# haoxiangsnr/Wave-U-Net-for-Speech-Enhancement

Measured on AMD Instinct MI355X. Metric: 16384-sample frames/sec fwd+bwd, 12-level Wave-U-Net, higher is better.
Workload: dtype f32 (levels >= 16 samples: 3 x f16 MFMA on hi/lo fp16 halves, fp32 accumulate; the rest f32 MFMA); 1 GPU; unet_basic 12-level, 16384-sample frames, batch=64 per GPU, fp32, training-mode forward + smooth_l1 + backward + fused HIP Adam step (BASELINE.json configs[2]; configs[3] when n_gpus>1); global_batch=64, frame=16384, parallelism=dp1

## Files before the change

### wave-u-net-for-speech-enhancement_amd/csrc/wunet_elementwise.h

```cpp
#pragma once
#include "wunet_dev.h"

struct PackDesc {
    const float* w;
    float* dst;
    int Cout, Cin, taps;
    int M;
    int CP;
    int mtiles;
    int transposed;
};

#define WUNET_MAX_CONV_LAYERS 34
struct PackTable { PackDesc d[WUNET_MAX_CONV_LAYERS]; };

static __global__ __launch_bounds__(WUNET_THREADS) void pack_weights_kernel(PackTable tab)
{
    const PackDesc& d = tab.d[blockIdx.y];
    const int total = d.mtiles * d.CP * d.taps * 16;
    const int kc = d.transposed ? d.Cout : d.Cin;
    for (int idx = blockIdx.x * WUNET_THREADS + threadIdx.x; idx < total; idx += gridDim.x * WUNET_THREADS) {
        const int i = idx & 15;
        int r = idx >> 4;
        const int t = r % d.taps; r /= d.taps;
        const int c = r % d.CP;
        const int mt = r / d.CP;
        const int m = mt * 16 + i;
        float v = 0.0f;
        if (m < d.M && c < kc) {
            v = d.transposed ? d.w[((size_t)c * d.Cin + m) * d.taps + (d.taps - 1 - t)]
                             : d.w[((size_t)m * d.Cin + c) * d.taps + t];
        }
        d.dst[idx] = v;
    }
}

template <int N>
__device__ __forceinline__ void block_sum(double (&a)[N], double* red)
{
    const int tid = threadIdx.x;
#pragma unroll
    for (int m = 32; m > 0; m >>= 1) {
#pragma unroll
        for (int k = 0; k < N; ++k) a[k] += wunet_shfl_xor_d(a[k], m);
    }
    __syncthreads();
    if ((tid & 63) == 0) {
#pragma unroll
        for (int k = 0; k < N; ++k) red[k * WUNET_WAVES + (tid >> 6)] = a[k];
    }
    __syncthreads();
#pragma unroll
    for (int k = 0; k < N; ++k)
        a[k] = (red[k * WUNET_WAVES] + red[k * WUNET_WAVES + 1]) + (red[k * WUNET_WAVES + 2] + red[k * WUNET_WAVES + 3]);
}

__device__ __forceinline__ void block_sum2(double& a, double& b, double* red)
{
    double v[2] = {a, b};
    block_sum<2>(v, red);
    a = v[0]; b = v[1];
}

struct RowPiece { size_t row, piece, beg, end; };
__device__ __forceinline__ RowPiece row_piece(size_t row, size_t piece, size_t plen, size_t len)
{
    const size_t beg = piece * plen;
    return RowPiece{row, piece, beg, beg + plen < len ? beg + plen : len};
}

__device__ __forceinline__ void block_max2(float& a, float& b, double* red)
{
    float* fr = reinterpret_cast<float*>(red);
    const int tid = threadIdx.x;
#pragma unroll
    for (int m = 32; m > 0; m >>= 1) {
        a = fmaxf(a, wunet_shfl_xor(a, m));
        b = fmaxf(b, wunet_shfl_xor(b, m));
    }
    __syncthreads();
    if ((tid & 63) == 0) {
        fr[tid >> 6] = a;
        fr[WUNET_WAVES + (tid >> 6)] = b;
    }
    __syncthreads();
    a = fmaxf(fmaxf(fr[0], fr[1]), fmaxf(fr[2], fr[3]));
    b = fmaxf(fmaxf(fr[WUNET_WAVES], fr[WUNET_WAVES + 1]), fmaxf(fr[WUNET_WAVES + 2], fr[WUNET_WAVES + 3]));
}

struct BnFwdArgs {
    const float* stats;
    int rows;
    const float* bias;
    const float* gamma;
    const float* beta;
    float* running_mean;
    float* running_var;
    long long* nbt;
    float* a;
    float* s;
    float* mean;
    float* rstd;
    int C;
    double count;
    int training;
};

struct BnFwdPre { float bias, gamma, beta, rmean, rvar; long long nbt; };
__device__ __forceinline__ BnFwdPre bn_finalize_preload(const BnFwdArgs& A, int c)
{
    BnFwdPre P;
    P.bias = A.bias[c]; P.gamma = A.gamma[c]; P.beta = A.beta[c]; P.rmean = A.running_mean[c]; P.rvar = A.running_var[c];
    P.nbt = c == 0 ? *A.nbt : 0;
    return P;
}
__device__ __forceinline__ void bn_finalize_core(const BnFwdArgs& A, int c, double s1, double s2, const BnFwdPre& P)
{
    const double m0 = s1 / A.count;
    double var = s2 / A.count - m0 * m0;
    var = var < 0.0 ? 0.0 : var;
    const double mean = m0 + (double)P.bias;
    const float rstd = (float)(1.0 / sqrt(var + 1e-5));
    const float a = P.gamma * rstd;
    const float sh = P.beta - (float)mean * a;
    A.a[c] = a;
    A.s[c] = sh;
    A.mean[c] = (float)mean;
    A.rstd[c] = rstd;
    const double unbiased = A.count > 1.0 ? var * A.count / (A.count - 1.0) : var;
    A.running_mean[c] = (float)(0.9 * (double)P.rmean + 0.1 * mean);
    A.running_var[c] = (float)(0.9 * (double)P.rvar + 0.1 * unbiased);
    if (c == 0) *A.nbt = P.nbt + 1;
}

__device__ __forceinline__ void bn_eval_core(const BnFwdArgs& A, int c)
{
    const float rstd = (float)(1.0 / sqrt((double)A.running_var[c] + 1e-5));
    const float a = A.gamma[c] * rstd;
    A.a[c] = a;
    A.s[c] = A.beta[c] - A.running_mean[c] * a;
}

struct BnEvalDesc { const float* gamma; const float* beta; const float* running_mean; const float* running_var; float* a; float* s; int C;
                    float* mean; float* rstd; };
struct BnEvalTable { BnEvalDesc d[WUNET_MAX_CONV_LAYERS]; };
static __global__ __launch_bounds__(WUNET_THREADS) void bn_eval_all_kernel(BnEvalTable T)
{
    const BnEvalDesc& d = T.d[blockIdx.y];
    const int c = blockIdx.x * WUNET_THREADS + threadIdx.x;
    if (c >= d.C) return;
    BnFwdArgs A{};
    A.gamma = d.gamma; A.beta = d.beta; A.running_mean = const_cast<float*>(d.running_mean); A.running_var = const_cast<float*>(d.running_var);
    A.a = d.a; A.s = d.s;
    bn_eval_core(A, c);
    if (d.mean) {
        const float rstd = (float)(1.0 / sqrt((double)d.running_var[c] + 1e-5)), a = d.gamma[c] * rstd;
        const float mu = d.running_mean[c], sh = d.beta[c] - mu * a;
        d.mean[c] = mu;
        d.rstd[c] = rstd;
    }
}

static __global__ __launch_bounds__(WUNET_THREADS) void bn_finalize_fwd_kernel(BnFwdArgs A)
{
    __shared__ double red[2 * WUNET_THREADS];
    const int c = blockIdx.x, tid = threadIdx.x;
    if (!A.training) {
        if (tid == 0) bn_eval_core(A, c);
        return;
    }
    const BnFwdPre P = bn_finalize_preload(A, c);
    double s1 = 0.0, s2 = 0.0;
    const float2* st = reinterpret_cast<const float2*>(A.stats) + (size_t)c * A.rows;
    int r = tid;
    for (; r + 3 * WUNET_THREADS < A.rows; r += 4 * WUNET_THREADS) {
        const float2 v0 = st[r], v1 = st[r + WUNET_THREADS], v2 = st[r + 2 * WUNET_THREADS], v3 = st[r + 3 * WUNET_THREADS];
        s1 += (double)v0.x; s2 += (double)v0.y;
        s1 += (double)v1.x; s2 += (double)v1.y;
        s1 += (double)v2.x; s2 += (double)v2.y;
        s1 += (double)v3.x; s2 += (double)v3.y;
    }
    for (; r < A.rows; r += WUNET_THREADS) {
        const float2 v = st[r];
        s1 += (double)v.x;
        s2 += (double)v.y;
    }
    block_sum2(s1, s2, red);
    if (tid == 0) bn_finalize_core(A, c, s1, s2, P);
}

__device__ __forceinline__ wunet_f4 wunet_sum_splits4(const float* p, int ksplit, size_t stride)
{
    wunet_f4 v = wunet_f4{0.f, 0.f, 0.f, 0.f};
    int k = 0;
    for (; k + 4 <= ksplit; k += 4) {
        const wunet_f4 t0 = wunet_ld4(p + (size_t)k * stride), t1 = wunet_ld4(p + (size_t)(k + 1) * stride);
        const wunet_f4 t2 = wunet_ld4(p + (size_t)(k + 2) * stride), t3 = wunet_ld4(p + (size_t)(k + 3) * stride);
#pragma unroll
        for (int j = 0; j < 4; ++j) { v[j] += t0[j]; v[j] += t1[j]; v[j] += t2[j]; v[j] += t3[j]; }
    }
    for (; k < ksplit; ++k) {
        const wunet_f4 t = wunet_ld4(p + (size_t)k * stride);
#pragma unroll
        for (int j = 0; j < 4; ++j) v[j] += t[j];
    }
    return v;
}

static __global__ __launch_bounds__(WUNET_THREADS) void conv_reduce_bn_kernel(BnFwdArgs A, const float* part, int ksplit,
                                                                        size_t split_stride, float* z, int B, int L, int logL,
                                                                        float* stats_rows, int Lt, float* xb)
{
    __shared__ double red[2 * WUNET_THREADS];
    const int c = blockIdx.x, tid = threadIdx.x;
    const float bias = A.bias[c];
    double s1 = 0.0, s2 = 0.0;
    const int total = B * L;
    if (!A.training) {
        const float ea = xb ? A.a[c] : 0.0f, es = xb ? A.s[c] : 0.0f;
        float m = 0.0f, m2 = 0.0f;
        if ((L & 3) == 0) {
            const int total4 = total >> 2;
            const int per = (total4 + gridDim.y - 1) / gridDim.y;
            const int beg = blockIdx.y * per, end = beg + per < total4 ? beg + per : total4;
            for (int p4 = beg + tid; p4 < end; p4 += WUNET_THREADS) {
                const int p = p4 << 2;
                const int b = p >> logL, l = p & (L - 1);
                const size_t off = ((size_t)b * A.C + c) * L + l;
                const wunet_f4 v = wunet_sum_splits4(part + off, ksplit, split_stride);
                wunet_f4 o;
#pragma unroll
                for (int j = 0; j < 4; ++j) {
                    o[j] = v[j] + bias;
                    m = fmaxf(m, fabsf(ea * o[j] + es));
                }
                wunet_st4(z + off, o);
            }
        } else {
            const int per = (total + gridDim.y - 1) / gridDim.y;
            const int beg = blockIdx.y * per, end = beg + per < total ? beg + per : total;
            for (int p = beg + tid; p < end; p += WUNET_THREADS) {
                const int b = p >> logL, l = p & (L - 1);
                const size_t off = ((size_t)b * A.C + c) * L + l;
                float v = 0.0f;
                for (int k = 0; k < ksplit; ++k) v += part[(size_t)k * split_stride + off];
                z[off] = v + bias;
                m = fmaxf(m, fabsf(ea * (v + bias) + es));
            }
        }
        if (xb) {
            block_max2(m, m2, red);
            if (tid == 0) wunet_atomic_absmax(xb, m);
        }
        return;
    }
    BnFwdPre P{};
    if (gridDim.y == 1) P = bn_finalize_preload(A, c);
    if ((L & 3) == 0) {
        const int total4 = total >> 2;
        const int per = (total4 + gridDim.y - 1) / gridDim.y;
        const int beg = blockIdx.y * per, end = beg + per < total4 ? beg + per : total4;
        for (int p4 = beg + tid; p4 < end; p4 += WUNET_THREADS) {
            const int p = p4 << 2;
            const int b = p >> logL, l = p & (L - 1);
            const size_t off = ((size_t)b * A.C + c) * L + l;
            const wunet_f4 v = wunet_sum_splits4(part + off, ksplit, split_stride);
            wunet_f4 o;
#pragma unroll
            for (int j = 0; j < 4; ++j) {
                o[j] = v[j] + bias;
                if (l + j < Lt) {
                    s1 += (double)v[j];
                    s2 += (double)v[j] * (double)v[j];
                }
            }
            wunet_st4(z + off, o);
        }
    } else {
        const int per = (total + gridDim.y - 1) / gridDim.y;
        const int beg = blockIdx.y * per, end = beg + per < total ? beg + per : total;
        for (int p = beg + tid; p < end; p += WUNET_THREADS) {
            const int b = p >> logL, l = p & (L - 1);
            const size_t off = ((size_t)b * A.C + c) * L + l;
            float v = 0.0f;
            for (int k = 0; k < ksplit; ++k) v += part[(size_t)k * split_stride + off];
            z[off] = v + bias;
            if (l < Lt) {
                s1 += (double)v;
                s2 += (double)v * (double)v;
            }
        }
    }
    block_sum2(s1, s2, red);
    if (tid == 0) {
        if (gridDim.y > 1) {
            float* st = stats_rows + ((size_t)c * gridDim.y + blockIdx.y) * 2;
            st[0] = (float)s1;
            st[1] = (float)s2;
        } else bn_finalize_core(A, c, s1, s2, P);
    }
}

static __global__ __launch_bounds__(WUNET_THREADS) void split_sum_kernel(const float* part, int ksplit, size_t n, float* out,
                                                                   const float* bias, int C, int logL)
{
    if ((n & 3) == 0 && (bias == nullptr || logL >= 2)) {
        const size_t n4 = n >> 2;
        for (size_t i4 = (size_t)blockIdx.x * WUNET_THREADS + threadIdx.x; i4 < n4; i4 += (size_t)gridDim.x * WUNET_THREADS) {
            const size_t i = i4 << 2;
            wunet_f4 v = wunet_sum_splits4(part + i, ksplit, n);
            const float bv = bias ? bias[(i >> logL) % (size_t)C] : 0.0f;
#pragma unroll
            for (int j = 0; j < 4; ++j) v[j] += bv;
            wunet_st4(out + i, v);
        }
        return;
    }
    for (size_t i = (size_t)blockIdx.x * WUNET_THREADS + threadIdx.x; i < n; i += (size_t)gridDim.x * WUNET_THREADS) {
        float v = 0.0f;
        for (int k = 0; k < ksplit; ++k) v += part[(size_t)k * n + i];
        out[i] = v + (bias ? bias[(i >> logL) % (size_t)C] : 0.0f);
    }
}

struct HeadFwdArgs {
    const float* z;
    const float* a;
    const float* s;
    const float* in;
    const float* wh;
    const float* bh;
    float* out;
    int B, C, T, logT;
};

static __global__ __launch_bounds__(WUNET_THREADS) void head_fwd_kernel(HeadFwdArgs A)
{
    const size_t total4 = ((size_t)A.B * A.T) >> 2;
    const float bh = A.bh[0], win = A.wh[A.C];
    for (size_t q4 = (size_t)blockIdx.x * WUNET_THREADS + threadIdx.x; q4 < total4; q4 += (size_t)gridDim.x * WUNET_THREADS) {
        const size_t p = q4 << 2;
        const size_t b = p >> A.logT, t = p & (size_t)(A.T - 1);
        const float* zr = A.z + b * A.C * A.T + t;
        const wunet_f4 xin = wunet_ld4(A.in + p);
        wunet_f4 acc = wunet_f4{bh, bh, bh, bh};
        int c = 0;
        for (; c + 24 <= A.C; c += 24) {
            wunet_f4 v[24];
#pragma unroll
            for (int e = 0; e < 24; ++e) v[e] = wunet_ld4(zr + (size_t)(c + e) * A.T);
#pragma unroll
            for (int e = 0; e < 24; ++e) {
                const float av = A.a[c + e], sv = A.s[c + e], wv = A.wh[c + e];
#pragma unroll
                for (int j = 0; j < 4; ++j) acc[j] += wv * wunet_lrelu(av * v[e][j] + sv);
            }
        }
        for (; c + 8 <= A.C; c += 8) {
            wunet_f4 v[8];
#pragma unroll
            for (int e = 0; e < 8; ++e) v[e] = wunet_ld4(zr + (size_t)(c + e) * A.T);
#pragma unroll
            for (int e = 0; e < 8; ++e) {
                const float av = A.a[c + e], sv = A.s[c + e], wv = A.wh[c + e];
#pragma unroll
                for (int j = 0; j < 4; ++j) acc[j] += wv * wunet_lrelu(av * v[e][j] + sv);
            }
        }
        for (; c < A.C; ++c) {
            const wunet_f4 v = wunet_ld4(zr + (size_t)c * A.T);
            const float av = A.a[c], sv = A.s[c], wv = A.wh[c];
#pragma unroll
            for (int j = 0; j < 4; ++j) acc[j] += wv * wunet_lrelu(av * v[j] + sv);
        }
        wunet_f4 o;
#pragma unroll
        for (int j = 0; j < 4; ++j) o[j] = tanhf(acc[j] + win * xin[j]);
        wunet_st4(A.out + p, o);
    }
}

struct HeadBwdArgs {
    const float* z; const float* a; const float* s; const float* in;
    const float* out; const float* gout;
    float* gh;
    float* part;
    int B, C, T, logT;
};

static __global__ __launch_bounds__(WUNET_THREADS) void head_bwd_kernel(HeadBwdArgs A)
{
    __shared__ double red[2 * WUNET_THREADS];
    const size_t total = (size_t)A.B * A.T;
    const size_t per = (total + gridDim.x - 1) / gridDim.x;
    const size_t beg = (size_t)blockIdx.x * per, end = beg + per < total ? beg + per : total;
    double sb = 0.0, sin_ = 0.0;
    size_t p = beg + threadIdx.x;
    for (; p + 3 * WUNET_THREADS < end; p += 4 * WUNET_THREADS) {
        float o[4], go[4], xi[4];
#pragma unroll
        for (int u = 0; u < 4; ++u) { o[u] = A.out[p + u * WUNET_THREADS]; go[u] = A.gout[p + u * WUNET_THREADS]; xi[u] = A.in[p + u * WUNET_THREADS]; }
#pragma unroll
        for (int u = 0; u < 4; ++u) {
            const float g = go[u] * (1.0f - o[u] * o[u]);
            A.gh[p + u * WUNET_THREADS] = g;
            sb += (double)g;
            sin_ += (double)g * (double)xi[u];
        }
    }
    for (; p < end; p += WUNET_THREADS) {
        const float o = A.out[p];
        const float g = A.gout[p] * (1.0f - o * o);
        A.gh[p] = g;
        sb += (double)g;
        sin_ += (double)g * (double)A.in[p];
    }
    block_sum2(sb, sin_, red);
    if (threadIdx.x == 0) {
        A.part[(size_t)blockIdx.x * 2] = (float)sin_;
        A.part[(size_t)blockIdx.x * 2 + 1] = (float)sb;
    }
}

static __global__ __launch_bounds__(WUNET_THREADS) void rows_sum_kernel(const float* part, int rows, int n, float* out0, int n0, float* out1)
{
    __shared__ double red[2 * WUNET_THREADS];
    const int j = blockIdx.x;
    double s = 0.0, dummy = 0.0;
    for (int r = threadIdx.x; r < rows; r += WUNET_THREADS) s += (double)part[(size_t)r * n + j];
    block_sum2(s, dummy, red);
    if (threadIdx.x == 0) {
        if (j < n0) out0[j] = (float)s; else out1[j - n0] = (float)s;
    }
}

struct BnBwdArgs {
    const float* part; int rows;
    const float* gamma; const float* mean; const float* rstd;
    float* dgamma; float* dbeta;
    float* dbias;
    float* k1; float* k2; float* k3;
    int C; double count;
    const float* pmax;
    float* bound;
    const float* e0rows;
    float* dw0;
    int frozen;
};

struct BnBwdFold { float k1, k2, k3, dgamma, dbeta, dbias, bound; };
__device__ __forceinline__ BnBwdFold bn_bwd_fold(float gamma, float rstd, float mean, double s1, double s2, double count, int frozen, float mg, float mz)
{
    const double m1 = frozen ? 0.0 : s1 / count, m2 = frozen ? 0.0 : s2 / count;
    const double a = (double)gamma * (double)rstd;
    BnBwdFold f;
    f.k1 = (float)a;
    f.k2 = (float)(-a * m2 * (double)rstd);
    f.k3 = (float)(a * m2 * (double)rstd * (double)mean - a * m1);
    f.dgamma = (float)s2;
    f.dbeta = (float)s1;
    f.dbias = frozen ? (float)(a * s1) : 0.0f;
    f.bound = (float)(fabs(a) * (double)mg + fabs(a * m2 * (double)rstd) * (double)mz + fabs(a * m1));
    return f;
}

enum { A_HEAD = 0, A_UP = 1, A_ENC = 2, A_UPH = 3 };

struct PassAArgs {
    const float* z;
    const float* a;
    const float* s;
    const float* mean;
    const float* rstd;
    float* gpre;
    float* part;
    float* pmax;
    float* hpart;
    union {
        struct {
            const float* g0;
            const float* g1;
            int Cg0;
        };
        WunetEncSrc enc;
    };
    size_t g1_stride;
    int g1_splits;
    int B, C, L, logL;
    float up_scale;
    int swap;
    int Lt;
    const float* sp;
    int ntiles, tpr;
    const float* x0; float* e0rows;
    const float* gamma; float* dgamma; float* dbeta; float* dbias; float* k1; float* k2; float* k3; double count;
    int frozen;
};

__device__ __forceinline__ void block_reduce_pass_a(double& s1, double& s2, double& s3, bool want3, float& mg, float& mz, double* red)
{
    const int tid = threadIdx.x;
#pragma unroll
    for (int m = 32; m > 0; m >>= 1) {
        s1 += wunet_shfl_xor_d(s1, m);
        s2 += wunet_shfl_xor_d(s2, m);
        if (want3) s3 += wunet_shfl_xor_d(s3, m);
        mg = fmaxf(mg, wunet_shfl_xor(mg, m));
        mz = fmaxf(mz, wunet_shfl_xor(mz, m));
    }
    if ((tid & 63) == 0) {
        const int w = tid >> 6;
        red[w] = s1; red[WUNET_WAVES + w] = s2; red[2 * WUNET_WAVES + w] = s3;
        red[3 * WUNET_WAVES + w] = (double)mg; red[4 * WUNET_WAVES + w] = (double)mz;
    }
    __syncthreads();
    s1 = (red[0] + red[1]) + (red[2] + red[3]);
    s2 = (red[WUNET_WAVES] + red[WUNET_WAVES + 1]) + (red[WUNET_WAVES + 2] + red[WUNET_WAVES + 3]);
    s3 = (red[2 * WUNET_WAVES] + red[2 * WUNET_WAVES + 1]) + (red[2 * WUNET_WAVES + 2] + red[2 * WUNET_WAVES + 3]);
    mg = fmaxf(fmaxf((float)red[3 * WUNET_WAVES], (float)red[3 * WUNET_WAVES + 1]), fmaxf((float)red[3 * WUNET_WAVES + 2], (float)red[3 * WUNET_WAVES + 3]));
    mz = fmaxf(fmaxf((float)red[4 * WUNET_WAVES], (float)red[4 * WUNET_WAVES + 1]), fmaxf((float)red[4 * WUNET_WAVES + 2], (float)red[4 * WUNET_WAVES + 3]));
}

template <int MODE, bool E0 = false>
struct PassALoads {
    wunet_f4 z, g;
    float e0, e1;
    float d[MODE == A_UP ? 13 : 1];
    wunet_f4 xw[E0 ? 5 : 1];
    size_t zi; int b, l;
};

template <int MODE, bool FUSE = false, bool G1S = false, bool E0 = false>
__global__ __launch_bounds__(WUNET_THREADS) void pass_a_kernel(PassAArgs A)
{
    static_assert(!E0 || (MODE == A_ENC && !FUSE && !G1S), "E0: the first layer's gradient assembly");
    __shared__ double red[5 * WUNET_WAVES];
    __shared__ float e0x[E0 ? WUNET_WAVES * 48 : 1];
    float w1[E0 ? 15 : 1], w2[E0 ? 15 : 1], w3[E0 ? 15 : 1];
    if (E0) {
#pragma unroll
        for (int k = 0; k < 15; ++k) w1[E0 ? k : 0] = w2[E0 ? k : 0] = w3[E0 ? k : 0] = 0.0f;
    }
    const int c = A.swap ? blockIdx.y : blockIdx.x;
    const unsigned by = A.swap ? blockIdx.x : blockIdx.y, ny = A.swap ? gridDim.x : gridDim.y;
    const size_t total4 = ((size_t)A.B * A.L) >> 2;
    const size_t per = (total4 + ny - 1) / ny;
    const size_t beg = (size_t)by * per, end = beg + per < total4 ? beg + per : total4;
    const float a = A.a[c], s = A.s[c], mu = A.mean[c], rstd = A.rstd[c];
    const float wh = MODE == A_HEAD ? A.g1[c] : 0.0f;
    const float gam = FUSE ? A.gamma[c] : 0.0f;
    double s1 = 0.0, s2 = 0.0, s3 = 0.0;
    float mg = 0.0f, mz = 0.0f;
    wunet_f4 keep_g = wunet_f4{0.f, 0.f, 0.f, 0.f}, keep_z = keep_g;
    size_t keep_i = 0;
    int keep_l = 0;
    bool have = false;

    auto load = [&](size_t q4, PassALoads<MODE, E0>& t) {
        const size_t p = q4 << 2;
        t.b = (int)(p >> A.logL); t.l = (int)(p & (size_t)(A.L - 1));
        const int b = t.b, l = t.l;
        t.zi = ((size_t)b * A.C + c) * A.L + l;
        t.z = wunet_ld4(A.z + t.zi);
        t.e0 = t.e1 = 0.0f;
        if (MODE == A_HEAD) t.g = wunet_ld4(A.g0 + (size_t)b * A.L + l);
        else if (MODE == A_UPH) {
            t.g = wunet_ld4(A.g0 + t.zi);
            const int tile = b * A.tpr + (l >> 7);
            t.e0 = A.sp[(size_t)c * A.ntiles + (tile > 0 ? tile - 1 : 0)];
            t.e1 = A.sp[((size_t)A.C + c) * A.ntiles + (tile + 1 < A.ntiles ? tile + 1 : tile)];
        }
        else if (MODE == A_ENC) {
            t.g = wunet_enc_skip4(A.enc, b, c, A.L, l);
            const float* ge = wunet_enc_half_at(A.enc, b, A.C, c, A.L, l);
            float e0, e1;
            if (G1S) {
                e0 = e1 = 0.0f;
                int k = 0;
                for (; k + 4 <= A.g1_splits; k += 4) {
                    const float2 t0 = *reinterpret_cast<const float2*>(ge + (size_t)k * A.g1_stride);
                    const float2 t1 = *reinterpret_cast<const float2*>(ge + (size_t)(k + 1) * A.g1_stride);
                    const float2 t2 = *reinterpret_cast<const float2*>(ge + (size_t)(k + 2) * A.g1_stride);
                    const float2 t3 = *reinterpret_cast<const float2*>(ge + (size_t)(k + 3) * A.g1_stride);
                    e0 += t0.x; e0 += t1.x; e0 += t2.x; e0 += t3.x;
                    e1 += t0.y; e1 += t1.y; e1 += t2.y; e1 += t3.y;
                }
                if (k < A.g1_splits) {
                    const int last = A.g1_splits - 1;
                    const float2 t0 = *reinterpret_cast<const float2*>(ge + (size_t)k * A.g1_stride);
                    const float2 t1 = *reinterpret_cast<const float2*>(ge + (size_t)(k + 1 < last ? k + 1 : last) * A.g1_stride);
                    const float2 t2 = *reinterpret_cast<const float2*>(ge + (size_t)(k + 2 < last ? k + 2 : last) * A.g1_stride);
                    e0 += t0.x; e1 += t0.y;
                    e0 += k + 1 <= last ? t1.x : 0.0f; e1 += k + 1 <= last ? t1.y : 0.0f;
                    e0 += k + 2 <= last ? t2.x : 0.0f; e1 += k + 2 <= last ? t2.y : 0.0f;
                }
            } else { const float2 tt = wunet_enc_half2(A.enc, b, A.C, c, A.L, l); e0 = tt.x; e1 = tt.y; }
            t.e0 = e0; t.e1 = e1;
            if (E0) {
                const float* xr = A.x0 + (size_t)b * A.L;
#pragma unroll
                for (int v = 0; v < 5; ++v) {
                    const int lv = l - 8 + 4 * v;
                    const bool ok = lv >= 0 && lv < A.L;
                    t.xw[E0 ? v : 0] = wunet_sel4(ok, wunet_ld4(xr + (ok ? lv : 0)));
                }
            }
        } else {
            const int Lo = 2 * A.L;
            const float* row = A.g0 + ((size_t)b * A.Cg0 + c) * Lo;
            const int j0 = 2 * l - 4;
#pragma unroll
            for (int v = 0; v < 3; ++v) {
                const int jv = j0 + 4 * v;
                const bool ok = jv >= 0 && jv < Lo;
                const wunet_f4 tt = wunet_sel4(ok, wunet_ld4(row + (ok ? jv : 0)));
                t.d[(MODE == A_UP ? 4 * v : 0)] = tt[0]; t.d[(MODE == A_UP ? 4 * v + 1 : 0)] = tt[1];
                t.d[(MODE == A_UP ? 4 * v + 2 : 0)] = tt[2]; t.d[(MODE == A_UP ? 4 * v + 3 : 0)] = tt[3];
            }
            t.d[MODE == A_UP ? 12 : 0] = (j0 + 12 < Lo) ? row[j0 + 12] : 0.0f;
            t.g = wunet_f4{0.f, 0.f, 0.f, 0.f};
        }
    };

    auto compute = [&](const PassALoads<MODE, E0>& t) {
        const int b = t.b, l = t.l;
        const wunet_f4 z = t.z;
        float g[4];
        if (MODE == A_HEAD) {
#pragma unroll
            for (int j = 0; j < 4; ++j) {
                g[j] = wh * t.g[j];
                s3 += (double)(t.g[j] * wunet_lrelu(a * z[j] + s));
            }
        } else if (MODE == A_UPH) {
            float* const gq = const_cast<float*>(A.g0) + t.zi;
            g[0] = t.g[0]; g[1] = t.g[1]; g[2] = t.g[2]; g[3] = t.g[3];
            const bool first = (l & 127) == 0 && l > 0, last = (l & 127) == 124 && l + 4 < A.L;
            g[0] += first ? t.e0 : 0.0f;
            g[3] += last ? t.e1 : 0.0f;
            if (first) gq[0] = g[0];
            if (last) gq[3] = g[3];
        } else if (MODE == A_ENC) {
            const wunet_f4 ge = wunet_enc_combine(t.g, float2{t.e0, t.e1});
            g[0] = ge[0]; g[1] = ge[1]; g[2] = ge[2]; g[3] = ge[3];
        } else {
            const int Lot = 2 * A.Lt;
            const float* d = t.d;
            const float dlast = t.d[MODE == A_UP ? 12 : 0];
            const int j0 = 2 * l - 4;
            g[0] = g[1] = g[2] = g[3] = 0.0f;
            bool fast = l >= 4 && l + 8 <= A.Lt;
            float c0[10], c1[10];
            if (fast) {
#pragma unroll
                for (int k = 3; k <= 12; ++k) {
                    int i0, i1;
                    wunet_up_coord(j0 + k, A.Lt, A.up_scale, i0, i1, c0[k - 3], c1[k - 3]);
                    fast = fast && i0 == ((j0 + k - 1) >> 1) && i1 == i0 + 1;
                }
            }
            if (fast) {
#pragma unroll
                for (int m = 0; m < 4; ++m) {
                    g[m] += c1[2 * m] * d[MODE == A_UP ? 2 * m + 3 : 0];
                    g[m] += c1[2 * m + 1] * d[MODE == A_UP ? 2 * m + 4 : 0];
                    g[m] += c0[2 * m + 2] * d[MODE == A_UP ? 2 * m + 5 : 0];
                    g[m] += c0[2 * m + 3] * (m == 3 ? dlast : d[MODE == A_UP ? (m == 3 ? 0 : 2 * m + 6) : 0]);
                }
            } else
#pragma unroll
            for (int k = 2; k <= 12; ++k) {
                const int j = j0 + k;
                const float dv = k < 12 ? d[MODE == A_UP ? (k < 12 ? k : 0) : 0] : dlast;
                if (j >= 0 && j < Lot) {
                    int i0, i1; float l0, l1;
                    wunet_up_coord(j, A.Lt, A.up_scale, i0, i1, l0, l1);
#pragma unroll
                    for (int m = 0; m < 4; ++m) {
                        const float w = (i0 == l + m ? l0 : 0.0f) + (i1 == l + m ? l1 : 0.0f);
                        g[m] += w * dv;
                    }
                }
            }
        }
        wunet_f4 go;
#pragma unroll
        for (int j = 0; j < 4; ++j) {
            float gv = wunet_lrelu_bwd(a, s, z[j], g[j]);
            const bool pad = l + j >= A.Lt;
            if (pad) gv = 0.0f;
            const float zc = pad ? 0.0f : z[j] - mu;
            go[j] = gv;
            s1 += (double)gv;
            s2 += (double)(gv * (zc * rstd));
            mg = fmaxf(mg, fabsf(gv));
            mz = fmaxf(mz, fabsf(zc));
        }
        if (E0) {
            float xs[20];
#pragma unroll
            for (int v = 0; v < 5; ++v) { xs[4 * v] = t.xw[E0 ? v : 0][0]; xs[4 * v + 1] = t.xw[E0 ? v : 0][1]; xs[4 * v + 2] = t.xw[E0 ? v : 0][2]; xs[4 * v + 3] = t.xw[E0 ? v : 0][3]; }
#pragma unroll
            for (int j = 0; j < 4; ++j) {
                const bool pad = l + j >= A.Lt;
                const float zz = pad ? 0.0f : z[j], one = pad ? 0.0f : 1.0f;
#pragma unroll
                for (int k = 0; k < 15; ++k) {
                    w1[E0 ? k : 0] = fmaf(go[j], xs[j + k + 1], w1[E0 ? k : 0]);
                    w2[E0 ? k : 0] = fmaf(zz, xs[j + k + 1], w2[E0 ? k : 0]);
                }
                if (c == 0) {
#pragma unroll
                    for (int k = 0; k < 15; ++k) w3[E0 ? k : 0] = fmaf(one, xs[j + k + 1], w3[E0 ? k : 0]);
                }
            }
        }
        if (FUSE) { keep_g = go; keep_z = z; keep_i = t.zi; keep_l = l; have = true; }
        else if (A.gpre) wunet_st4(A.gpre + t.zi, go);
    };

    for (size_t q4 = beg + threadIdx.x; q4 < end; q4 += 2 * WUNET_THREADS) {
        PassALoads<MODE, E0> t0, t1;
        const bool two = !FUSE && q4 + WUNET_THREADS < end;
        load(q4, t0);
        if (!FUSE) load(two ? q4 + WUNET_THREADS : q4, t1);
        compute(t0);
        if (two) compute(t1);
    }
    const bool want_max = A.pmax != nullptr;
    if (E0) {
#pragma unroll
        for (int q = 0; q < 45; ++q) {
            float v = q < 15 ? w1[E0 ? q : 0] : q < 30 ? w2[E0 ? q - 15 : 0] : w3[E0 ? q - 30 : 0];
            v = wunet_row16_sum(v);
            v += wunet_shfl_xor(v, 16);
            v += wunet_shfl_xor(v, 32);
            if ((threadIdx.x & 63) == 0) e0x[E0 ? (threadIdx.x >> 6) * 48 + q : 0] = v;
        }
        __syncthreads();
        if (threadIdx.x < 45) {
            const int q = threadIdx.x;
            A.e0rows[((size_t)by * A.C + c) * 48 + q] = (e0x[E0 ? q : 0] + e0x[E0 ? 48 + q : 0]) + (e0x[E0 ? 96 + q : 0] + e0x[E0 ? 144 + q : 0]);
        }
    }
    block_reduce_pass_a(s1, s2, s3, MODE == A_HEAD, mg, mz, red);
    if (FUSE) {
        const BnBwdFold f = bn_bwd_fold(gam, rstd, mu, (double)(float)s1, (double)(float)s2, A.count, A.frozen, 0.0f, 0.0f);
        if (threadIdx.x == 0) {
            A.dgamma[c] = f.dgamma;
            A.dbeta[c] = f.dbeta;
            A.dbias[c] = f.dbias;
            A.k1[c] = f.k1; A.k2[c] = f.k2; A.k3[c] = f.k3;
        }
        if (have) {
            wunet_f4 o;
#pragma unroll
            for (int j = 0; j < 4; ++j) o[j] = keep_l + j < A.Lt ? wunet_gz(f.k1, f.k2, f.k3, keep_g[j], keep_z[j]) : 0.0f;
            wunet_st4(A.gpre + keep_i, o);
        }
        return;
    }
    if (threadIdx.x == 0) {
        float* pr = A.part + ((size_t)by * A.C + c) * 2;
        pr[0] = (float)s1;
        pr[1] = (float)s2;
        if (want_max) {
            float* pm = A.pmax + ((size_t)by * A.C + c) * 2;
            pm[0] = mg;
            pm[1] = mz;
        }
        if (MODE == A_HEAD && A.hpart) A.hpart[(size_t)by * A.C + c] = (float)s3;
    }
}

static __global__ __launch_bounds__(WUNET_THREADS) void bn_finalize_bwd_kernel(BnBwdArgs A)
{
    __shared__ double red[5 * WUNET_WAVES];
    const int c = blockIdx.x, tid = threadIdx.x;
    const float gam = A.gamma[c], rs = A.rstd[c], mu = A.mean[c];
    double s1 = 0.0, s2 = 0.0, s3 = 0.0;
    float mg = 0.0f, mz = 0.0f;
    for (int r = tid; r < A.rows; r += WUNET_THREADS) {
        const float2 pr = *reinterpret_cast<const float2*>(A.part + ((size_t)r * A.C + c) * 2);
        float2 pm = float2{0.0f, 0.0f};
        if (A.pmax) pm = *reinterpret_cast<const float2*>(A.pmax + ((size_t)r * A.C + c) * 2);
        s1 += (double)pr.x;
        s2 += (double)pr.y;
        mg = fmaxf(mg, pm.x);
        mz = fmaxf(mz, pm.y);
    }
    block_reduce_pass_a(s1, s2, s3, false, mg, mz, red);
    const BnBwdFold f = bn_bwd_fold(gam, rs, mu, s1, s2, A.count, A.frozen, mg, mz);
    if (tid == 0) {
        A.dgamma[c] = f.dgamma;
        A.dbeta[c] = f.dbeta;
        A.dbias[c] = f.dbias;
        A.k1[c] = f.k1;
        A.k2[c] = f.k2;
        A.k3[c] = f.k3;
        if (A.pmax) A.bound[c] = f.bound;
    }
    if (A.e0rows) {
        __shared__ double e0s[48];
        if (tid < 45) {
            double t = 0.0;
            for (int r0 = 0; r0 < A.rows; r0 += 32) {
                float v[32];
#pragma unroll
                for (int r = 0; r < 32; ++r) v[r] = A.e0rows[((size_t)(r0 + r < A.rows ? r0 + r : 0) * A.C + (tid < 30 ? c : 0)) * 48 + tid];
#pragma unroll
                for (int r = 0; r < 32; ++r) if (r0 + r < A.rows) t += (double)v[r];
            }
            e0s[tid] = t;
        }
        __syncthreads();
        if (tid < 15) A.dw0[c * 15 + tid] = (float)((double)f.k1 * e0s[tid] + (double)f.k2 * e0s[15 + tid] + (double)f.k3 * e0s[30 + tid]);
    }
}

static __global__ __launch_bounds__(WUNET_THREADS) void wgrad_reduce_kernel(const float* part, int splits, size_t n, float* dw)
{
    __shared__ double red[16][16][4];
    const int og = threadIdx.x & 15, sl = threadIdx.x >> 4;
    const size_t n4 = n >> 2;
    for (size_t base = (size_t)blockIdx.x * 16; base < n4; base += (size_t)gridDim.x * 16) {
        const size_t i = base + og;
        double t0 = 0.0, t1 = 0.0, t2 = 0.0, t3 = 0.0;
        if (i < n4) {
            int r = sl;
            for (; r + 7 * 16 < splits; r += 8 * 16) {
                float a0 = 0.f, a1 = 0.f, a2 = 0.f, a3 = 0.f;
#pragma unroll
                for (int k = 0; k < 8; ++k) {
                    const wunet_f4 v = wunet_ld4(part + (size_t)(r + k * 16) * n + 4 * i);
                    a0 += v[0]; a1 += v[1]; a2 += v[2]; a3 += v[3];
                }
                t0 += (double)a0; t1 += (double)a1; t2 += (double)a2; t3 += (double)a3;
            }
            for (; r < splits; r += 16) {
                const wunet_f4 v = wunet_ld4(part + (size_t)r * n + 4 * i);
                t0 += (double)v[0]; t1 += (double)v[1]; t2 += (double)v[2]; t3 += (double)v[3];
            }
        }
        __syncthreads();
        red[sl][og][0] = t0; red[sl][og][1] = t1; red[sl][og][2] = t2; red[sl][og][3] = t3;
        __syncthreads();
        if (sl == 0 && i < n4) {
            double u0 = 0.0, u1 = 0.0, u2 = 0.0, u3 = 0.0;
#pragma unroll
            for (int k = 0; k < 16; ++k) { u0 += red[k][og][0]; u1 += red[k][og][1]; u2 += red[k][og][2]; u3 += red[k][og][3]; }
            wunet_f4 o;
            o[0] = (float)u0; o[1] = (float)u1; o[2] = (float)u2; o[3] = (float)u3;
            wunet_st4(dw + 4 * i, o);
        }
    }
    for (size_t i = (n4 << 2) + (size_t)blockIdx.x * WUNET_THREADS + threadIdx.x; i < n; i += (size_t)gridDim.x * WUNET_THREADS) {
        double tot = 0.0;
        for (int r = 0; r < splits; ++r) tot += (double)part[(size_t)r * n + i];
        dw[i] = (float)tot;
    }
}

template <int K>
__global__ __launch_bounds__(WUNET_THREADS) void conv_first_kernel(const float* x, const float* w, const float* bias, float* out,
                                                                    float* stats, int B, int Cout, int L, int logL,
                                                                    const float* ev_a, const float* ev_s, float* xrows, int Lt)
{
    constexpr int PAD = K / 2, NX = ((8 + 4 + PAD + 3) / 4) * 4;
    static_assert(PAD <= 8 && NX >= 8 + 4 + PAD, "window");
    const int lane = threadIdx.x & 63, wave = threadIdx.x >> 6;
    const size_t p = ((size_t)blockIdx.x * WUNET_THREADS + threadIdx.x) * 4;
    const int b = (int)(p >> logL), l0 = (int)(p & (size_t)(L - 1));
    const bool live = b < B;
    const bool counted = live && l0 < Lt;
    float xv[NX];
#pragma unroll
    for (int v = 0; v < NX / 4; ++v) {
        const int l = l0 - 8 + 4 * v;
        const bool ok = live && l >= 0 && l < L;
        const wunet_f4 t = wunet_sel4(ok, wunet_ld4(x + (ok ? (size_t)b * L + l : 0)));
        xv[4 * v] = t[0]; xv[4 * v + 1] = t[1]; xv[4 * v + 2] = t[2]; xv[4 * v + 3] = t[3];
    }
    const size_t rows = (size_t)gridDim.x * WUNET_WAVES, row = (size_t)blockIdx.x * WUNET_WAVES + wave;
    float amax = 0.0f;
#pragma unroll 2
    for (int co = 0; co < Cout; ++co) {
        const float* wr = w + (size_t)co * K;
        wunet_f4 acc = wunet_f4{0.f, 0.f, 0.f, 0.f};
#pragma unroll
        for (int t = 0; t < K; ++t) {
            const float wv = wr[t];
#pragma unroll
            for (int j = 0; j < 4; ++j) acc[j] = fmaf(wv, xv[8 - PAD + t + j], acc[j]);
        }
        float s1 = counted ? (acc[0] + acc[1]) + (acc[2] + acc[3]) : 0.0f;
        float s2 = counted ? (acc[0] * acc[0] + acc[1] * acc[1]) + (acc[2] * acc[2] + acc[3] * acc[3]) : 0.0f;
        if (live) {
            const float bv = bias ? bias[co] : 0.0f;
            wunet_f4 o;
#pragma unroll
            for (int j = 0; j < 4; ++j) o[j] = acc[j] + bv;
            wunet_st4(out + ((size_t)b * Cout + co) * L + l0, o);
            if (xrows) {
                const float ea = ev_a[co], es = ev_s[co];
#pragma unroll
                for (int j = 0; j < 4; ++j) amax = fmaxf(amax, fabsf(ea * o[j] + es));
            }
        }
        if (stats) {
            s1 = wunet_row16_sum(s1);
            s2 = wunet_row16_sum(s2);
#pragma unroll
            for (int m = 16; m < 64; m <<= 1) {
                s1 += wunet_shfl_xor(s1, m);
                s2 += wunet_shfl_xor(s2, m);
            }
            if (lane == 0) {
                float* stp = stats + ((size_t)co * rows + row) * 2;
                stp[0] = s1;
                stp[1] = s2;
            }
        }
    }
    if (xrows) {
        __shared__ float xm[WUNET_WAVES];
#pragma unroll
        for (int m = 1; m < 64; m <<= 1) amax = fmaxf(amax, wunet_shfl_xor(amax, m));
        if (lane == 0) xm[wave] = amax;
        __syncthreads();
        if (threadIdx.x == 0) wunet_atomic_absmax(xrows, fmaxf(fmaxf(xm[0], xm[1]), fmaxf(xm[2], xm[3])));
    }
}

struct PrepArgs {
    const float* z0; const float* a0; const float* s0;
    const float* z1; const float* a1; const float* s1;
    float* x;
    int B, C0, C1, L, logL;
    float up_scale;
    int Lt;
};

static __global__ __launch_bounds__(WUNET_THREADS) void prep_decim_kernel(PrepArgs A)
{
    const int l4n = A.L >> 2;
    const size_t total = (size_t)A.B * A.C0 * l4n;
    for (size_t i = (size_t)blockIdx.x * WUNET_THREADS + threadIdx.x; i < total; i += (size_t)gridDim.x * WUNET_THREADS) {
        const size_t row = i >> (A.logL - 2);
        const int l4 = (int)(i & (size_t)(l4n - 1));
        const int c = (int)(row % (size_t)A.C0);
        const float a = A.a0[c], s = A.s0[c];
        const float4* src = reinterpret_cast<const float4*>(A.z0 + row * (size_t)(2 * A.L) + 8 * l4);
        const float4 u = src[0], v = src[1];
        float4 o;
        o.x = wunet_lrelu(a * u.x + s); o.y = wunet_lrelu(a * u.z + s);
        o.z = wunet_lrelu(a * v.x + s); o.w = wunet_lrelu(a * v.z + s);
        if (4 * l4 + 3 >= A.Lt) {
            if (4 * l4 >= A.Lt) o.x = 0.0f;
            if (4 * l4 + 1 >= A.Lt) o.y = 0.0f;
            if (4 * l4 + 2 >= A.Lt) o.z = 0.0f;
            o.w = 0.0f;
        }
        reinterpret_cast<float4*>(A.x)[i] = o;
    }
}

static __global__ __launch_bounds__(WUNET_THREADS) void prep_upcat_kernel(PrepArgs A, int cbeg, int cend)
{
    const int l4n = A.L >> 2, C = A.C0 + A.C1, Lh = A.L >> 1, nc = cend - cbeg;
    const size_t total = (size_t)A.B * nc * l4n;
    for (size_t i = (size_t)blockIdx.x * WUNET_THREADS + threadIdx.x; i < total; i += (size_t)gridDim.x * WUNET_THREADS) {
        const size_t row = i >> (A.logL - 2);
        const int l4 = (int)(i & (size_t)(l4n - 1));
        const int b = (int)(row / (size_t)nc), c = cbeg + (int)(row - (size_t)b * nc);
        float4 o;
        if (c < A.C0) {
            const float a = A.a0[c], s = A.s0[c];
            const float* zr = A.z0 + ((size_t)b * A.C0 + c) * Lh;
            float r[4];
#pragma unroll
            for (int j = 0; j < 4; ++j) {
                int i0, i1; float l0, l1;
                wunet_up_coord(4 * l4 + j, A.Lt >> 1, A.up_scale, i0, i1, l0, l1);
                r[j] = l0 * wunet_lrelu(a * zr[i0] + s) + l1 * wunet_lrelu(a * zr[i1] + s);
            }
            o.x = r[0]; o.y = r[1]; o.z = r[2]; o.w = r[3];
        } else {
            const int cs = c - A.C0;
            const float a = A.a1[cs], s = A.s1[cs];
            const float4 v = reinterpret_cast<const float4*>(A.z1 + ((size_t)b * A.C1 + cs) * A.L)[l4];
            o.x = wunet_lrelu(a * v.x + s); o.y = wunet_lrelu(a * v.y + s);
            o.z = wunet_lrelu(a * v.z + s); o.w = wunet_lrelu(a * v.w + s);
        }
        if (4 * l4 + 3 >= A.Lt) {
            if (4 * l4 >= A.Lt) o.x = 0.0f;
            if (4 * l4 + 1 >= A.Lt) o.y = 0.0f;
            if (4 * l4 + 2 >= A.Lt) o.z = 0.0f;
            o.w = 0.0f;
        }
        reinterpret_cast<float4*>(A.x + ((size_t)b * C + c) * A.L)[l4] = o;
    }
}

static __global__ __launch_bounds__(WUNET_THREADS) void gz_materialize_kernel(const float* g, const float* z, const float* k1, const float* k2,
                                                                        const float* k3, int C, int logL, size_t n4, float* gz, int Lt)
{
    for (size_t i = (size_t)blockIdx.x * WUNET_THREADS + threadIdx.x; i < n4; i += (size_t)gridDim.x * WUNET_THREADS) {
        const int c = (int)((i >> (logL - 2)) % (size_t)C);
        const float a = k1[c], b = k2[c], d = k3[c];
        const float4 gv = reinterpret_cast<const float4*>(g)[i], zv = reinterpret_cast<const float4*>(z)[i];
        float4 o;
        o.x = wunet_gz(a, b, d, gv.x, zv.x); o.y = wunet_gz(a, b, d, gv.y, zv.y);
        o.z = wunet_gz(a, b, d, gv.z, zv.z); o.w = wunet_gz(a, b, d, gv.w, zv.w);
        const int l = (int)((i << 2) & (((size_t)1 << logL) - 1));
        if (l + 3 >= Lt) {
            if (l >= Lt) o.x = 0.0f;
            if (l + 1 >= Lt) o.y = 0.0f;
            if (l + 2 >= Lt) o.z = 0.0f;
            o.w = 0.0f;
        }
        reinterpret_cast<float4*>(gz)[i] = o;
    }
}

static __global__ __launch_bounds__(WUNET_THREADS) void crop_windows_kernel(const float* mix_flat, const float* clean_flat, const long long* starts,
                                                                            long long total, int length, float* mix, float* clean)
{
    const int b = blockIdx.y;
    long long s0 = starts[b];
    if (s0 < 0) s0 = 0;
    if (s0 > total - length) s0 = total - length;
    const int j0 = (blockIdx.x * WUNET_THREADS + threadIdx.x) * 4;
    if (j0 >= length) return;
    const float* ms = mix_flat + s0 + j0;
    const float* cs = clean_flat + s0 + j0;
    float* md = mix + (size_t)b * length + j0;
    float* cd = clean + (size_t)b * length + j0;
    if (j0 + 4 <= length && (length & 3) == 0) {
        const wunet_f4 m = {ms[0], ms[1], ms[2], ms[3]};
        const wunet_f4 c = {cs[0], cs[1], cs[2], cs[3]};
        wunet_st4(md, m);
        wunet_st4(cd, c);
    } else {
        for (int k = 0; k < 4 && j0 + k < length; ++k) { md[k] = ms[k]; cd[k] = cs[k]; }
    }
}

static __global__ __launch_bounds__(WUNET_THREADS) void fill_kernel(float* p, size_t n, float v)
{
    for (size_t i = (size_t)blockIdx.x * WUNET_THREADS + threadIdx.x; i < n; i += (size_t)gridDim.x * WUNET_THREADS) p[i] = v;
}

__device__ __forceinline__ float loss_term(int kind, float d)
{
    if (kind == 0) return d * d;
    const float ad = fabsf(d);
    if (kind == 1) return ad;
    return ad < 1.0f ? 0.5f * d * d : ad - 0.5f;
}
__device__ __forceinline__ float loss_dterm(int kind, float d)
{
    if (kind == 0) return 2.0f * d;
    const float sg = (d > 0.0f ? 1.0f : 0.0f) - (d < 0.0f ? 1.0f : 0.0f);
    if (kind == 1) return sg;
    return fabsf(d) < 1.0f ? d : sg;
}

static __global__ __launch_bounds__(WUNET_THREADS) void loss_partial_kernel(int kind, const float* clean, const float* enh, size_t n, double* part)
{
    __shared__ double red[WUNET_WAVES];
    double s[1] = {0.0};
    const size_t stride = (size_t)gridDim.x * WUNET_THREADS;
    size_t i = (size_t)blockIdx.x * WUNET_THREADS + threadIdx.x;
    for (; i + 3 * stride < n; i += 4 * stride) {
        float e[4], c[4];
#pragma unroll
        for (int u = 0; u < 4; ++u) { e[u] = enh[i + u * stride]; c[u] = clean[i + u * stride]; }
#pragma unroll
        for (int u = 0; u < 4; ++u) s[0] += (double)loss_term(kind, e[u] - c[u]);
    }
    for (; i < n; i += stride) s[0] += (double)loss_term(kind, enh[i] - clean[i]);
    block_sum<1>(s, red);
    if (threadIdx.x == 0) part[blockIdx.x] = s[0];
}

static __global__ __launch_bounds__(WUNET_THREADS) void loss_final_kernel(const double* part, int rows, size_t n, float* loss)
{
    __shared__ double red[WUNET_WAVES];
    double s[1] = {0.0};
    for (int r = threadIdx.x; r < rows; r += WUNET_THREADS) s[0] += part[r];
    block_sum<1>(s, red);
    if (threadIdx.x == 0) *loss = (float)(s[0] / (double)n);
}

static __global__ __launch_bounds__(WUNET_THREADS) void loss_bwd_kernel(int kind, const float* clean, const float* enh, const float* gscale, size_t n, float* genh)
{
    const float sc = gscale[0] / (float)n;
    const size_t stride = (size_t)gridDim.x * WUNET_THREADS;
    size_t i = (size_t)blockIdx.x * WUNET_THREADS + threadIdx.x;
    for (; i + 3 * stride < n; i += 4 * stride) {
        float e[4], c[4];
#pragma unroll
        for (int u = 0; u < 4; ++u) { e[u] = enh[i + u * stride]; c[u] = clean[i + u * stride]; }
#pragma unroll
        for (int u = 0; u < 4; ++u) genh[i + u * stride] = sc * loss_dterm(kind, e[u] - c[u]);
    }
    for (; i < n; i += stride) genh[i] = sc * loss_dterm(kind, enh[i] - clean[i]);
}

#define WUNET_ADAM_MAX 64
struct AdamTable {
    float* p[WUNET_ADAM_MAX];
    const float* g[WUNET_ADAM_MAX];
    float* m[WUNET_ADAM_MAX];
    float* v[WUNET_ADAM_MAX];
    unsigned n[WUNET_ADAM_MAX];
};

static __global__ __launch_bounds__(WUNET_THREADS) void adam_kernel(AdamTable T, float one_minus_b1, float b2, float one_minus_b2,
                                                              float bc2_sqrt, float eps, float step_size, float gscale,
                                                              const float* hyper)
{
    if (hyper) { step_size = hyper[0]; bc2_sqrt = hyper[1]; }
    const int t = blockIdx.y;
    float* p = T.p[t];
    const float* g = T.g[t];
    float* m = T.m[t];
    float* v = T.v[t];
    const unsigned n = T.n[t];
    for (unsigned i = blockIdx.x * WUNET_THREADS + threadIdx.x; i < n; i += gridDim.x * WUNET_THREADS) {
        const float gi = gscale == 1.0f ? g[i] : g[i] * gscale;
        float mi = m[i], vi = v[i];
        mi = mi + one_minus_b1 * (gi - mi);
        vi = vi * b2 + one_minus_b2 * gi * gi;
        m[i] = mi;
        v[i] = vi;
        const float denom = sqrtf(vi) / bc2_sqrt + eps;
        p[i] = p[i] - step_size * (mi / denom);
    }
}

static __global__ void adam_hyper_kernel(long long* step, double lr, double beta1, double beta2, float* hyper)
{
    const long long t = *step + 1;
    *step = t;
    const double bc1 = 1.0 - pow(beta1, (double)t), bc2 = 1.0 - pow(beta2, (double)t);
    hyper[0] = (float)(lr / bc1);
    hyper[1] = (float)sqrt(bc2);
}

#define WUNET_HYPER_STEP_SIZE 0
#define WUNET_HYPER_BC2_SQRT 1
#define WUNET_HYPER_CLIP 2
#define WUNET_HYPER_NORM 3
#define WUNET_HYPER_DECAY 4

static __global__ __launch_bounds__(WUNET_THREADS) void grad_sqnorm_partial_kernel(AdamTable T, float gscale, double* part)
{
    __shared__ double red[WUNET_WAVES];
    const int t = blockIdx.y;
    const float* g = T.g[t];
    const unsigned n = T.n[t];
    const double gs = (double)gscale;
    double s[1] = {0.0};
    const size_t stride = (size_t)gridDim.x * WUNET_THREADS;
    size_t i = (size_t)blockIdx.x * WUNET_THREADS + threadIdx.x;
    for (; i + 3 * stride < n; i += 4 * stride) {
        float e[4];
#pragma unroll
        for (int u = 0; u < 4; ++u) e[u] = g[i + u * stride];
#pragma unroll
        for (int u = 0; u < 4; ++u) { const double x = gs * (double)e[u]; s[0] += x * x; }
    }
    for (; i < n; i += stride) { const double x = gs * (double)g[i]; s[0] += x * x; }
    block_sum<1>(s, red);
    if (threadIdx.x == 0) part[(size_t)blockIdx.y * gridDim.x + blockIdx.x] = s[0];
}

static __global__ __launch_bounds__(WUNET_THREADS) void adam_hyper_ex_kernel(long long* step_dev, long long step, double lr, const double* lr_dev,
                                                                       double beta1, double beta2, double weight_decay, double max_norm,
                                                                       const double* part, int n_part, float* hyper)
{
    __shared__ double red[WUNET_WAVES];
    double s[1] = {0.0};
    int r = threadIdx.x;
    for (; r + 3 * WUNET_THREADS < n_part; r += 4 * WUNET_THREADS) {
        double e[4];
#pragma unroll
        for (int u = 0; u < 4; ++u) e[u] = part[r + u * WUNET_THREADS];
#pragma unroll
        for (int u = 0; u < 4; ++u) s[0] += e[u];
    }
    for (; r < n_part; r += WUNET_THREADS) s[0] += part[r];
    block_sum<1>(s, red);
    if (threadIdx.x != 0) return;
    long long t = step;
    if (step_dev) {
        t = *step_dev + 1;
        *step_dev = t;
    }
    if (lr_dev) lr = *lr_dev;
    const double bc1 = 1.0 - pow(beta1, (double)t), bc2 = 1.0 - pow(beta2, (double)t);
    double norm = 0.0, clip = 1.0;
    if (n_part > 0) {
        norm = sqrt(s[0]);
        const double c = max_norm / (norm + 1e-6);
        clip = c > 1.0 ? 1.0 : c;
    }
    hyper[WUNET_HYPER_STEP_SIZE] = (float)(lr / bc1);
    hyper[WUNET_HYPER_BC2_SQRT] = (float)sqrt(bc2);
    hyper[WUNET_HYPER_CLIP] = (float)clip;
    hyper[WUNET_HYPER_NORM] = (float)norm;
    hyper[WUNET_HYPER_DECAY] = (float)(1.0 - lr * weight_decay);
}

__device__ __forceinline__ float adam_update(float p, float step_size, float q)
{
#ifdef WUNET_EMU
    return p - step_size * q;
#else
    return __builtin_fmaf(-step_size, q, p);
#endif
}

static __global__ __launch_bounds__(WUNET_THREADS) void adam_ex_kernel(AdamTable T, float one_minus_b1, float b2, float one_minus_b2,
                                                                 float eps, float gscale, const float* hyper)
{
    const float step_size = hyper[WUNET_HYPER_STEP_SIZE], bc2_sqrt = hyper[WUNET_HYPER_BC2_SQRT];
    const float factor = gscale * hyper[WUNET_HYPER_CLIP], decay = hyper[WUNET_HYPER_DECAY];
    const int t = blockIdx.y;
    float* p = T.p[t];
    const float* g = T.g[t];
    float* m = T.m[t];
    float* v = T.v[t];
    const unsigned n = T.n[t];
    for (unsigned i = blockIdx.x * WUNET_THREADS + threadIdx.x; i < n; i += gridDim.x * WUNET_THREADS) {
#ifdef __clang__
#pragma clang fp contract(off)
#endif
        const float gi = factor == 1.0f ? g[i] : g[i] * factor;
        float mi = m[i], vi = v[i];
        mi = mi + one_minus_b1 * (gi - mi);
        vi = vi * b2 + one_minus_b2 * gi * gi;
        m[i] = mi;
        v[i] = vi;
        const float denom = sqrtf(vi) / bc2_sqrt + eps;
        float pi = p[i];
        if (decay != 1.0f) pi = pi * decay;
        p[i] = adam_update(pi, step_size, mi / denom);
    }
}
```

Before: 12790 frames/s.

## Defer UPH edge stores, specialize single-row blocks, prefetch e0 rows in BN finalize

In the UPH pass-A path, the boundary gradient writes back into g0 are deferred. Eight iterations of edge values are buffered and written only after a waitcnt on outstanding loads, so the stores no longer serialize against in-flight loads to the same buffer. Blocks whose range lies within one batch row get a specialization that skips the per-element row division. The BN finalize kernel now issues up to 128 e0row loads per lane before the partial-sum loop, so that latency overlaps the main reduction; this adds register pressure and relies on a hand-coded waitcnt immediate.

```diff
diff --git a/wave-u-net-for-speech-enhancement_amd/csrc/wunet_elementwise.h b/wave-u-net-for-speech-enhancement_amd/csrc/wunet_elementwise.h
--- a/wave-u-net-for-speech-enhancement_amd/csrc/wunet_elementwise.h
+++ b/wave-u-net-for-speech-enhancement_amd/csrc/wunet_elementwise.h
@@ -530,6 +530,16 @@
     size_t zi; int b, l;
 };
 
+__device__ __forceinline__ bool uph_first(int l) { return (l & 127) == 0 && l > 0; }
+__device__ __forceinline__ bool uph_last(int l, int L) { return (l & 127) == 124 && l + 4 < L; }
+template <bool V> struct WunetFlag { static constexpr bool value = V; };
+#define WUNET_UPH_KEEP 8
+#ifdef WUNET_EMU
+#define wunet_loads_landed() ((void)0)
+#else
+#define wunet_loads_landed() __builtin_amdgcn_s_waitcnt(0x0F70)
+#endif
+
 template <int MODE, bool FUSE = false, bool G1S = false, bool E0 = false>
 __global__ __launch_bounds__(WUNET_THREADS) void pass_a_kernel(PassAArgs A)
 {
@@ -556,9 +566,10 @@
     int keep_l = 0;
     bool have = false;
 
-    auto load = [&](size_t q4, PassALoads<MODE, E0>& t) {
+    const int b_row = (int)((beg << 2) >> A.logL);
+    auto load = [&](auto row1, size_t q4, PassALoads<MODE, E0>& t) {
         const size_t p = q4 << 2;
-        t.b = (int)(p >> A.logL); t.l = (int)(p & (size_t)(A.L - 1));
+        t.b = decltype(row1)::value ? b_row : (int)(p >> A.logL); t.l = (int)(p & (size_t)(A.L - 1));
         const int b = t.b, l = t.l;
         t.zi = ((size_t)b * A.C + c) * A.L + l;
         t.z = wunet_ld4(A.z + t.zi);
@@ -622,7 +633,7 @@
         }
     };
 
-    auto compute = [&](const PassALoads<MODE, E0>& t) {
+    auto compute = [&](const PassALoads<MODE, E0>& t, float& edge) {
         const int b = t.b, l = t.l;
         const wunet_f4 z = t.z;
         float g[4];
@@ -633,13 +644,11 @@
                 s3 += (double)(t.g[j] * wunet_lrelu(a * z[j] + s));
             }
         } else if (MODE == A_UPH) {
-            float* const gq = const_cast<float*>(A.g0) + t.zi;
             g[0] = t.g[0]; g[1] = t.g[1]; g[2] = t.g[2]; g[3] = t.g[3];
-            const bool first = (l & 127) == 0 && l > 0, last = (l & 127) == 124 && l + 4 < A.L;
+            const bool first = uph_first(l), last = uph_last(l, A.L);
             g[0] += first ? t.e0 : 0.0f;
             g[3] += last ? t.e1 : 0.0f;
-            if (first) gq[0] = g[0];
-            if (last) gq[3] = g[3];
+            edge = first ? g[0] : g[3];
         } else if (MODE == A_ENC) {
             const wunet_f4 ge = wunet_enc_combine(t.g, float2{t.e0, t.e1});
             g[0] = ge[0]; g[1] = ge[1]; g[2] = ge[2]; g[3] = ge[3];
@@ -719,14 +728,54 @@
         else if (A.gpre) wunet_st4(A.gpre + t.zi, go);
     };
 
-    for (size_t q4 = beg + threadIdx.x; q4 < end; q4 += 2 * WUNET_THREADS) {
-        PassALoads<MODE, E0> t0, t1;
-        const bool two = !FUSE && q4 + WUNET_THREADS < end;
-        load(q4, t0);
-        if (!FUSE) load(two ? q4 + WUNET_THREADS : q4, t1);
-        compute(t0);
-        if (two) compute(t1);
-    }
+    auto store_edge = [&](auto row1, size_t q4, float v) {
+        const size_t p = q4 << 2;
+        const int b = decltype(row1)::value ? b_row : (int)(p >> A.logL), l = (int)(p & (size_t)(A.L - 1));
+        float* const gq = const_cast<float*>(A.g0) + ((size_t)b * A.C + c) * A.L + l;
+        if (uph_first(l)) gq[0] = v;
+        if (uph_last(l, A.L)) gq[3] = v;
+    };
+
+    auto trips = [&](auto row1) {
+        if (MODE == A_UPH) {
+            for (size_t qc = beg + threadIdx.x; qc < end; qc += WUNET_UPH_KEEP * WUNET_THREADS) {
+                float ek[WUNET_UPH_KEEP];
+#pragma unroll
+                for (int u = 0; u < WUNET_UPH_KEEP; ++u) ek[u] = 0.0f;
+#pragma unroll
+                for (int u = 0; u < WUNET_UPH_KEEP; u += 2) {
+                    const size_t q4 = qc + (size_t)u * WUNET_THREADS;
+                    if (q4 < end) {
+                        PassALoads<MODE, E0> t0, t1;
+                        const bool two = q4 + WUNET_THREADS < end;
+                        load(row1, q4, t0);
+                        load(row1, two ? q4 + WUNET_THREADS : q4, t1);
+                        compute(t0, ek[u]);
+                        if (two) compute(t1, ek[u + 1]);
+                    }
+                }
+                wunet_loads_landed();
+#pragma unroll
+                for (int u = 0; u < WUNET_UPH_KEEP; ++u) {
+                    const size_t q4 = qc + (size_t)u * WUNET_THREADS;
+                    if (q4 < end) store_edge(row1, q4, ek[u]);
+                }
+            }
+        } else {
+            for (size_t q4 = beg + threadIdx.x; q4 < end; q4 += 2 * WUNET_THREADS) {
+                PassALoads<MODE, E0> t0, t1;
+                float none;
+                const bool two = !FUSE && q4 + WUNET_THREADS < end;
+                load(row1, q4, t0);
+                if (!FUSE) load(row1, two ? q4 + WUNET_THREADS : q4, t1);
+                compute(t0, none);
+                if (two) compute(t1, none);
+            }
+        }
+    };
+    const bool one_row = !FUSE && !G1S && (MODE == A_UPH || MODE == A_ENC) && beg < end && b_row == (int)(((end << 2) - 1) >> A.logL);
+    if (one_row) trips(WunetFlag<true>{});
+    else trips(WunetFlag<false>{});
     const bool want_max = A.pmax != nullptr;
     if (E0) {
 #pragma unroll
@@ -773,11 +822,21 @@
     }
 }
 
+#define WUNET_E0_FIN_ROWS 128
 static __global__ __launch_bounds__(WUNET_THREADS) void bn_finalize_bwd_kernel(BnBwdArgs A)
 {
     __shared__ double red[5 * WUNET_WAVES];
     const int c = blockIdx.x, tid = threadIdx.x;
     const float gam = A.gamma[c], rs = A.rstd[c], mu = A.mean[c];
+    __shared__ double e0s[48];
+    const bool e0w = A.e0rows != nullptr && tid < 64;
+    const bool e0all = e0w && A.rows >= WUNET_E0_FIN_ROWS;
+    const size_t e0col = (size_t)(tid < 30 ? c : 0) * 48 + (tid < 45 ? tid : 0), e0row = (size_t)A.C * 48;
+    float ev[WUNET_E0_FIN_ROWS];
+    if (e0all) {
+#pragma unroll
+        for (int r = 0; r < WUNET_E0_FIN_ROWS; ++r) ev[r] = A.e0rows[e0col + (size_t)r * e0row];
+    }
     double s1 = 0.0, s2 = 0.0, s3 = 0.0;
     float mg = 0.0f, mz = 0.0f;
     for (int r = tid; r < A.rows; r += WUNET_THREADS) {
@@ -789,6 +848,23 @@
         mg = fmaxf(mg, pm.x);
         mz = fmaxf(mz, pm.y);
     }
+    if (e0w && tid < 45) {
+        double t = 0.0;
+        int r0 = 0;
+        if (e0all) {
+#pragma unroll
+            for (int r = 0; r < WUNET_E0_FIN_ROWS; ++r) t += (double)ev[r];
+            r0 = WUNET_E0_FIN_ROWS;
+        }
+        for (; r0 < A.rows; r0 += 32) {
+            float v[32];
+#pragma unroll
+            for (int r = 0; r < 32; ++r) v[r] = A.e0rows[e0col + (size_t)(r0 + r < A.rows ? r0 + r : 0) * e0row];
+#pragma unroll
+            for (int r = 0; r < 32; ++r) if (r0 + r < A.rows) t += (double)v[r];
+        }
+        e0s[tid] = t;
+    }
     block_reduce_pass_a(s1, s2, s3, false, mg, mz, red);
     const BnBwdFold f = bn_bwd_fold(gam, rs, mu, s1, s2, A.count, A.frozen, mg, mz);
     if (tid == 0) {
@@ -800,22 +876,7 @@
         A.k3[c] = f.k3;
         if (A.pmax) A.bound[c] = f.bound;
     }
-    if (A.e0rows) {
-        __shared__ double e0s[48];
-        if (tid < 45) {
-            double t = 0.0;
-            for (int r0 = 0; r0 < A.rows; r0 += 32) {
-                float v[32];
-#pragma unroll
-                for (int r = 0; r < 32; ++r) v[r] = A.e0rows[((size_t)(r0 + r < A.rows ? r0 + r : 0) * A.C + (tid < 30 ? c : 0)) * 48 + tid];
-#pragma unroll
-                for (int r = 0; r < 32; ++r) if (r0 + r < A.rows) t += (double)v[r];
-            }
-            e0s[tid] = t;
-        }
-        __syncthreads();
-        if (tid < 15) A.dw0[c * 15 + tid] = (float)((double)f.k1 * e0s[tid] + (double)f.k2 * e0s[15 + tid] + (double)f.k3 * e0s[30 + tid]);
-    }
+    if (A.e0rows && tid < 15) A.dw0[c * 15 + tid] = (float)((double)f.k1 * e0s[tid] + (double)f.k2 * e0s[15 + tid] + (double)f.k3 * e0s[30 + tid]);
 }
 
 static __global__ __launch_bounds__(WUNET_THREADS) void wgrad_reduce_kernel(const float* part, int splits, size_t n, float* dw)
```

Result: no change. 12750 frames/s, median of 2 (-0.3%).
